# dtarb/TauDEM

Hardware: AMD Instinct MI355X
Metric: Mcells/s (PitRemove->D8FlowDir->AreaD8 pipeline) (higher is better)
Workload: dtype f32

## Files before the change

taudem_amd/csrc/aread8.hip:

```cpp
#include "context.hpp"
#include "device_common.hpp"
#include "d8_sweep.hpp"
#include "flats.hpp"
#include "strips.hpp"

#include <cstdlib>
#include <cstring>

namespace {
using namespace tdxk;

constexpr int32_t CNT_NOT_PART = 0x40000000;
constexpr int32_t CNT_SOURCE = -1;
constexpr int32_t CNT_DONE = -2;

constexpr int16_t P_OUTSIDE = 16, P_SINK = 32;

enum { D8X_SUM = 0, D8X_MAX = 1, D8X_MIN = 2 };
struct D8Expr { int mode; float out_nodata; };
__device__ __forceinline__ bool d8_participates(int16_t p, int16_t nodata) { return !is_nodata_s(p, nodata) && ((p >= 0 && p <= 8) || p == P_SINK); }

__device__ __forceinline__ int d8_indegree(const int16_t* __restrict__ P, int nx, int ny, int x, int y, int16_t nodata) {
    int cnt = 0;
#pragma unroll
// ... 175 lines not shown
                if (xn >= 0 && xn < nx && yn >= y_own0 && yn < y_own1) {
                    const size_t n = size_t(yn) * size_t(nx) + size_t(xn);
                    drain_stores();
                    const int32_t old = __hip_atomic_fetch_sub(&cnt[n], 1, __ATOMIC_ACQ_REL, __HIP_MEMORY_SCOPE_AGENT);
                    if (old == 1) ad8_walk_from(n, P, Wt, w_nodata, nx, ny, y_own0, y_own1, nodata, contcheck, cnt, A, ex);
                }
            }
        }
    }
    const unsigned long long m = __ballot(ch);
    if ((threadIdx.x & 63) == 0 && m) atomicAdd(nchanged, (unsigned long long)__popcll(m));
}


constexpr int TS = 64;
constexpr int TH = TS + 2;
static_assert(TS == 64, "S_TGT() shifts by 6");
constexpr uint32_t NODE_DEAD = 0xFFFFFFFEu;
constexpr uint32_t NEXT_NONE = 0xFFFFFFFFu;
constexpr uint32_t NEXT_REMOTE_UP = 0xFFFFFFFDu;
constexpr uint32_t NEXT_REMOTE_DOWN = 0xFFFFFFFCu;
constexpr unsigned long long BOX_VALID = 1ull << 63;
constexpr float BIG_MARK = -2.0f;

static __global__ __launch_bounds__(256) void ad8_init_kernel(unsigned long long* __restrict__ d_cnt, uint32_t* __restrict__ node_indeg, uint32_t* __restrict__ node_next, size_t nnodes,
                                                              unsigned long long* __restrict__ boxes, uint8_t* __restrict__ delivered, size_t nx) {
    const size_t i = size_t(blockIdx.x) * 256 + threadIdx.x;
    if (i < 8) d_cnt[i] = 0ull;
    if (i < nnodes) { node_indeg[i] = 0xFFFFFFFFu; node_next[i] = 0xFFFFFFFFu; }
    if (i < 4 * nx) boxes[i] = 0ull;
    if (i < 2 * nx) delivered[i] = 0;
}
struct Ad8Geom {
    int nx, ny_arr, y0, y1, tiles_x, tiles_y;
    uint32_t nnodes_local;
};
__device__ __forceinline__ int rows_valid(const Ad8Geom& g, int ty) { const int r = g.y1 - (g.y0 + ty * TS); return r < TS ? r : TS; }

__device__ __forceinline__ unsigned lw_pack(unsigned cnt, unsigned arr, unsigned con, unsigned poi, unsigned indeg) {
    return cnt | (arr << 13) | (con << 17) | (poi << 21) | (indeg << 25);
}
__device__ __forceinline__ unsigned lw_cnt(unsigned w) { return w & 0x1FFFu; }
__device__ __forceinline__ unsigned lw_arr(unsigned w) { return (w >> 13) & 15u; }
__device__ __forceinline__ unsigned lw_con(unsigned w) { return (w >> 17) & 15u; }
__device__ __forceinline__ unsigned lw_poi(unsigned w) { return (w >> 21) & 15u; }
__device__ __forceinline__ unsigned lw_indeg(unsigned w) { return (w >> 25) & 15u; }
__device__ __forceinline__ unsigned long long nw_pack(unsigned cnt, unsigned arr, unsigned con, unsigned poi) {
    return (unsigned long long)cnt | ((unsigned long long)arr << 32) | ((unsigned long long)con << 42) | ((unsigned long long)poi << 52);
}
__device__ __forceinline__ unsigned nw_arr(unsigned long long w) { return unsigned(w >> 32) & 1023u; }
__device__ __forceinline__ unsigned nw_con(unsigned long long w) { return unsigned(w >> 42) & 1023u; }
__device__ __forceinline__ unsigned nw_poi(unsigned long long w) { return unsigned(w >> 52) & 1023u; }
__device__ __forceinline__ uint32_t cw_pack(unsigned cnt, bool con, bool poi) { return cnt | (con ? 1u << 30 : 0u) | (poi ? 1u << 31 : 0u); }

__device__ __forceinline__ int perim_pos(int lx, int ly, int rv) {
    if (ly == 0) return lx;
    if (ly == rv - 1) return 64 + lx;
    if (lx == 0) return 128 + (ly - 1);
    return 190 + (ly - 1);
}
__device__ __forceinline__ uint32_t node_id(const Ad8Geom& g, int gx, int gy) {
    if (gy < g.y0) return g.nnodes_local + uint32_t(gx);
    if (gy >= g.y1) return g.nnodes_local + uint32_t(g.nx) + uint32_t(gx);
    const int ty = (gy - g.y0) / TS, ly = (gy - g.y0) % TS;
    return uint32_t(ty * g.tiles_x + gx / TS) * 256u + uint32_t(perim_pos(gx % TS, ly, rows_valid(g, ty)));
}


constexpr unsigned OH_NODATA = 0x8000u, OH_SINK = 0x4000u, OH_DIRS = 0x1FEu, OH_PART = 0x1FFu | OH_SINK;
__device__ __forceinline__ unsigned p_onehot(int v, int nodata) {
    const unsigned sel = v == nodata ? 15u : (v == int(P_SINK) ? 14u : (unsigned(v) <= 8u ? unsigned(v) : 31u));
    return (1u << sel) & (0x1FFu | OH_SINK | OH_NODATA);
}
__device__ __forceinline__ void stage_p_onehot(const int16_t* __restrict__ P, int nx, int ny_arr, int x0, int ya0, int16_t nodata, uint16_t* sO) {
    constexpr int NIT = (TH * TH + 255) / 256, HALF = (NIT + 1) / 2;
#pragma unroll
    for (int b = 0; b < 2; b++) {
        int16_t v[HALF];
        unsigned ok = 0;
#pragma unroll
        for (int i = 0; i < HALF; i++) {
            const int e = int(threadIdx.x) + (b * HALF + i) * 256, ec = e < TH * TH ? e : TH * TH - 1;
            const int ly = ec / TH, lx = ec - ly * TH;
            const int gx = x0 + lx - 1, gy = ya0 + ly - 1;
            const int gxc = gx < 0 ? 0 : (gx >= nx ? nx - 1 : gx), gyc = gy < 0 ? 0 : (gy >= ny_arr ? ny_arr - 1 : gy);
            v[i] = P[size_t(gyc) * size_t(nx) + size_t(gxc)];
            if (gx == gxc && gy == gyc) ok |= 1u << i;
        }
#pragma unroll
        for (int i = 0; i < HALF; i++) {
            const int e = int(threadIdx.x) + (b * HALF + i) * 256;
            if (b * HALF + i < NIT && e < TH * TH) sO[e] = uint16_t(((ok >> i) & 1u) ? p_onehot(int(v[i]), int(nodata)) : OH_NODATA);
        }
        __builtin_amdgcn_sched_barrier(0);
    }
}
__device__ __forceinline__ bool in_tile(int lx, int ly, int rv) { return lx >= 0 && lx < TS && ly >= 0 && ly < rv; }

__device__ __forceinline__ bool ring_cell(int j, int rv, int& hx, int& hy) {
    if (j < TH) { hx = j - 1; hy = -1; return true; }
    if (j < 2 * TH) { hx = j - TH - 1; hy = rv; return true; }
    j -= 2 * TH;
    if (j < rv) { hx = -1; hy = j; return true; }
    j -= rv;
    if (j < rv) { hx = TS; hy = j; return true; }
    return false;
// ... 117 lines not shown
    }
    __syncthreads();
    AD8_MARK(3);
    for (int j = tid; j < 4 * TH; j += 256) {
        int hx, hy;
        if (!ring_cell(j, rv, hx, hy)) continue;
        const unsigned dirs = sRing[j] & OH_DIRS;
        if (!dirs) continue;
        const int ph = __ffs(int(dirs)) - 1;
        const int vx = hx + d1(ph), vy = hy + d2(ph);
        if (!in_tile(vx, vy, rv)) continue;
        int cur = vy * TS + vx, hops = 0;
        if (lw_indeg(sAcc[cur]) == 15u) continue;
        while (S_TGT(cur) >= 0 && hops < TS * TS) { cur = S_TGT(cur); hops++; }
        uint32_t nxt = NEXT_NONE;
        if (S_TGT(cur) == -2) {
            const int pp = perim_pos(cur % TS, cur / TS, rv);
            atomicAdd(&sIn[pp], 1u);
            nxt = uint32_t(tile) * 256u + uint32_t(pp);
        }
        node_next[node_id(g, x0 + hx, ya0 + hy)] = nxt;
    }
    __syncthreads();
    AD8_MARK(4);
#pragma unroll
    for (int r = 0; r < 16; r++) {
        const int ly = ry0 + r, c = ly * TS + lx;
        const int gx = x0 + lx, gy = ya0 + ly;
        if (gx >= g.nx || ly >= rv) continue;
        const unsigned w = sAcc[c];
        const bool part = lw_indeg(w) != 15u;
        const bool complete = part && lw_arr(w) == lw_indeg(w);
        cellw[size_t(gy) * size_t(g.nx) + size_t(gx)] = part ? cw_pack(lw_cnt(w), lw_con(w) != 0u, lw_poi(w) != 0u || !complete) : 0u;
        if (part && tgt[r] == -2) {
            const int pp = perim_pos(lx, ly, rv);
            const uint32_t nid = uint32_t(tile) * 256u + uint32_t(pp);
            node_acc[nid] = nw_pack(lw_cnt(w), 0u, lw_con(w) ? 1u : 0u, lw_poi(w) ? 1u : 0u);
            node_indeg[nid] = complete ? sIn[pp] : NODE_DEAD;
            const int tgy = gy + (((exit_up >> r) & 1u) ? -1 : (((exit_down >> r) & 1u) ? 1 : 0));
            if (tgy < g.y0) node_next[nid] = NEXT_REMOTE_UP;
            else if (tgy >= g.y1) node_next[nid] = NEXT_REMOTE_DOWN;
        }
    }
#undef S_TGT
    if (DBG) {
        __syncthreads();
        AD8_MARK(5);
        if (tid == 0)
            for (int i = 0; i < 5; i++) atomicAdd(&g_ad8_dbg[i], tcs[i + 1] - tcs[i]);
    }
#undef AD8_MARK
}

__device__ __forceinline__ bool stage_p_raw(const int16_t* __restrict__ P, int nx, int ny_arr, int x0, int ya0, int16_t nodata, uint8_t* sC) {
    constexpr int NIT = (TH * TH + 255) / 256, HALF = (NIT + 1) / 2;
    bool bad = false;
#pragma unroll
    for (int b = 0; b < 2; b++) {
        int16_t v[HALF];
        unsigned ok = 0;
#pragma unroll
        for (int i = 0; i < HALF; i++) {
            const int e = int(threadIdx.x) + (b * HALF + i) * 256, ec = e < TH * TH ? e : TH * TH - 1;
            const int ly = ec / TH, lx = ec - ly * TH;
            const int gx = x0 + lx - 1, gy = ya0 + ly - 1;
            const int gxc = gx < 0 ? 0 : (gx >= nx ? nx - 1 : gx), gyc = gy < 0 ? 0 : (gy >= ny_arr ? ny_arr - 1 : gy);
            v[i] = P[size_t(gyc) * size_t(nx) + size_t(gxc)];
            if (gx == gxc && gy == gyc) ok |= 1u << i;
        }
#pragma unroll
        for (int i = 0; i < HALF; i++) {
            const int e = int(threadIdx.x) + (b * HALF + i) * 256;
            if (b * HALF + i < NIT && e < TH * TH) {
                const bool good = ((ok >> i) & 1u) && v[i] != nodata && unsigned(int(v[i]) - 1) < 8u;
                sC[e] = good ? uint8_t(v[i]) : uint8_t(0);
                bad |= !good;
            }
        }
        __builtin_amdgcn_sched_barrier(0);
    }
    return bad;
}

__device__ unsigned long long g_ad8_dbg_fast[8];
constexpr int AD8_MAX_ROUNDS = 12;
template <bool DBG>
__global__ __launch_bounds__(256, 6) void ad8_tile_fast_kernel(const int16_t* __restrict__ P, Ad8Geom g, int16_t nodata,
                                                            uint32_t* __restrict__ cellw, unsigned long long* __restrict__ node_acc,
                                                            uint32_t* __restrict__ node_indeg, uint32_t* __restrict__ node_next,
                                                            uint32_t* __restrict__ redo, unsigned long long* __restrict__ nredo) {
    unsigned long long tcs[6];
#define AD8_MARK(i) do { if (DBG) tcs[i] = clock64(); } while (0)
    AD8_MARK(0);
    __shared__ int16_t sT[TS * TS];
    __shared__ unsigned sAcc[TS * TS];
    __shared__ unsigned sIn[256];
    __shared__ unsigned sVote[3][4];
    static_assert(TH * TH <= int(sizeof(int16_t)) * TS * TS, "the staged codes fit the pointer table");
    uint8_t* const sC = reinterpret_cast<uint8_t*>(sT);
    const int tile = blockIdx.x;
    const int tx = tile % g.tiles_x, ty = tile / g.tiles_x;
    const int x0 = tx * TS, ya0 = g.y0 + ty * TS, rv = rows_valid(g, ty);
    const int tid = threadIdx.x, lx = tid & 63, ry0 = (tid >> 6) * 16, wave = tid >> 6;
    bool bad = rv != TS || x0 < 1 || x0 + TS >= g.nx || ya0 < 1 || ya0 + TS >= g.ny_arr;
    if (!bad) bad = stage_p_raw(P, g.nx, g.ny_arr, x0, ya0, nodata, sC);
    sIn[tid] = 0u;
    const bool wave_bad = __ballot(bad) != 0ull;
    if (lx == 0) sVote[0][wave] = wave_bad ? 1u : 0u;
    __syncthreads();
    if ((sVote[0][0] | sVote[0][1] | sVote[0][2] | sVote[0][3]) != 0u) {
        if (tid == 0) redo[atomicAdd(nredo, 1ull)] = uint32_t(tile);
        return;
    }
    AD8_MARK(1);
    unsigned exits = 0, exit_up = 0, exit_down = 0;
    int16_t ptr[16];
#pragma unroll
    for (int r = 0; r < 16; r++) {
        const int ly = ry0 + r;
        const int p = sC[(ly + 1) * TH + lx + 1];
        const int tlx = lx + d1(p), tly = ly + d2(p);
        const bool in = in_tile(tlx, tly, TS);
        ptr[r] = int16_t(in ? tly * TS + tlx : -2);
        if (!in) {
            exits |= 1u << r;
            if (d2(p) < 0) exit_up |= 1u << r;
            if (d2(p) > 0) exit_down |= 1u << r;
        }
    }
    int ent[2];
#pragma unroll
    for (int k = 0; k < 2; k++) {
        const int j = tid + 256 * k;
        int hx, hy;
        ent[k] = -1;
        if (j < 4 * TH && ring_cell(j, TS, hx, hy)) {
            const int ph = sC[(hy + 1) * TH + hx + 1];
            const int vx = hx + d1(ph), vy = hy + d2(ph);
            if (in_tile(vx, vy, TS)) ent[k] = vy * TS + vx;
        }
    }
    __syncthreads();
#pragma unroll
    for (int r = 0; r < 16; r++) {
        sT[(ry0 + r) * TS + lx] = ptr[r];
        sAcc[(ry0 + r) * TS + lx] = 1u;
    }
    __syncthreads();
    AD8_MARK(2);
    uint32_t ent_next[2];
#pragma unroll
    for (int k = 0; k < 2; k++) {
        ent_next[k] = NEXT_NONE;
        if (ent[k] < 0) continue;
        int cur = ent[k], hops = 0;
        while (sT[cur] >= 0 && hops < TS * TS) { cur = sT[cur]; hops++; }
        if (sT[cur] == -2) {
            const int pp = perim_pos(cur % TS, cur / TS, TS);
            atomicAdd(&sIn[pp], 1u);
            ent_next[k] = uint32_t(tile) * 256u + uint32_t(pp);
        }
    }
    __syncthreads();
    AD8_MARK(3);
    unsigned acc[16];
    unsigned live = ~exits & 0xFFFFu;
#pragma unroll
    for (int r = 0; r < 16; r++) acc[r] = 1u;
    int rounds = 0;
    for (;;) {
        int nn[16];
#pragma unroll
        for (int r = 0; r < 16; r++) nn[r] = sT[((live >> r) & 1u) ? int(ptr[r]) : (ry0 + r) * TS + lx];
#pragma unroll
        for (int r = 0; r < 16; r++)
            if ((live >> r) & 1u) (void)__hip_atomic_fetch_add(&sAcc[ptr[r]], acc[r], __ATOMIC_RELAXED, __HIP_MEMORY_SCOPE_WORKGROUP);
        __syncthreads();
#pragma unroll
        for (int r = 0; r < 16; r++)
            if ((live >> r) & 1u) {
                const int c = (ry0 + r) * TS + lx;
                ptr[r] = int16_t(nn[r]);
                sT[c] = int16_t(nn[r]);
                if (nn[r] < 0) live &= ~(1u << r);
                else acc[r] = sAcc[c];
            }
        rounds++;
        const bool wave_live = __ballot(live != 0u) != 0ull;
        if (lx == 0) sVote[1 + (rounds & 1)][wave] = wave_live ? 1u : 0u;
        __syncthreads();
        const unsigned* v = sVote[1 + (rounds & 1)];
        if ((v[0] | v[1] | v[2] | v[3]) == 0u) break;
        if (rounds == AD8_MAX_ROUNDS) {
            if (tid == 0) redo[atomicAdd(nredo, 1ull)] = uint32_t(tile);
            return;
        }
    }
    AD8_MARK(4);
#pragma unroll
    for (int k = 0; k < 2; k++) {
        const int j = tid + 256 * k;
        int hx, hy;
        if (ent[k] >= 0 && ring_cell(j, TS, hx, hy)) node_next[node_id(g, x0 + hx, ya0 + hy)] = ent_next[k];
    }
#pragma unroll
    for (int r = 0; r < 16; r++) {
        const int ly = ry0 + r, c = ly * TS + lx;
        const int gx = x0 + lx, gy = ya0 + ly;
        const unsigned cnt = sAcc[c];
        cellw[size_t(gy) * size_t(g.nx) + size_t(gx)] = cw_pack(cnt, false, false);
        if ((exits >> r) & 1u) {
            const int pp = perim_pos(lx, ly, TS);
            const uint32_t nid = uint32_t(tile) * 256u + uint32_t(pp);
            node_acc[nid] = nw_pack(cnt, 0u, 0u, 0u);
            node_indeg[nid] = sIn[pp];
            const int tgy = gy + (((exit_up >> r) & 1u) ? -1 : (((exit_down >> r) & 1u) ? 1 : 0));
            if (tgy < g.y0) node_next[nid] = NEXT_REMOTE_UP;
            else if (tgy >= g.y1) node_next[nid] = NEXT_REMOTE_DOWN;
        }
    }
    if (DBG) {
        __syncthreads();
        AD8_MARK(5);
        if (tid == 0) {
            for (int i = 0; i < 5; i++) atomicAdd(&g_ad8_dbg_fast[i], tcs[i + 1] - tcs[i]);
            atomicAdd(&g_ad8_dbg_fast[5], (unsigned long long)rounds);
            atomicAdd(&g_ad8_dbg_fast[6], 1ull);
        }
    }
#undef AD8_MARK
}

__device__ __forceinline__ void forest_walk_from(uint32_t u, unsigned long long w, const Ad8Geom& g, unsigned long long* __restrict__ node_acc,
                                                 const uint32_t* __restrict__ node_indeg, const uint32_t* __restrict__ node_next,
                                                 unsigned long long* __restrict__ outbox) {
    uint32_t n = node_next[u];
    for (;;) {
        if (n == NEXT_NONE) return;
        if (n == NEXT_REMOTE_UP || n == NEXT_REMOTE_DOWN) {
            const uint32_t tile = u >> 8, pos = u & 255u;
            const uint32_t gx = (tile % uint32_t(g.tiles_x)) * TS + (pos & 63u);
            outbox[(n == NEXT_REMOTE_UP ? 0u : uint32_t(g.nx)) + gx] = (w & ~BOX_VALID) | BOX_VALID;
            return;
        }
        const uint32_t nn = node_next[n], ind = node_indeg[n];
        const unsigned long long add = nw_pack(unsigned(w), 1u, nw_con(w) ? 1u : 0u, nw_poi(w) ? 1u : 0u);
        const unsigned long long nw = __hip_atomic_fetch_add(&node_acc[n], add, __ATOMIC_RELAXED, __HIP_MEMORY_SCOPE_AGENT) + add;
        if (nw_arr(nw) != ind) return;
        u = n; w = nw; n = nn;
    }
}

__global__ __launch_bounds__(256) void ad8_forest_walk_kernel(Ad8Geom g, unsigned long long* __restrict__ node_acc, const uint32_t* __restrict__ node_indeg,
                                                              const uint32_t* __restrict__ node_next, unsigned long long* __restrict__ outbox) {
    const size_t i = size_t(blockIdx.x) * 256 + threadIdx.x;
    if (i >= g.nnodes_local || node_indeg[i] != 0u) return;
    forest_walk_from(uint32_t(i), node_acc[i], g, node_acc, node_indeg, node_next, outbox);
}

__global__ __launch_bounds__(256) void ad8_forest_deliver_kernel(Ad8Geom g, const unsigned long long* __restrict__ inbox, uint8_t* __restrict__ delivered,
                                                                 unsigned long long* __restrict__ node_acc, uint32_t* __restrict__ node_indeg,
                                                                 const uint32_t* __restrict__ node_next, unsigned long long* __restrict__ outbox,
                                                                 unsigned long long* __restrict__ ndelivered) {
    const int i = blockIdx.x * 256 + threadIdx.x;
    bool did = false;
    if (i < 2 * g.nx) {
        const unsigned long long b = inbox[i];
        if ((b & BOX_VALID) && !delivered[i]) {
            delivered[i] = 1;
            did = true;
            const uint32_t hn = g.nnodes_local + uint32_t(i);
            const unsigned long long w = b & ~BOX_VALID;
            const unsigned long long hw = nw_pack(unsigned(w), 0u, nw_con(w) ? 1u : 0u, nw_poi(w) ? 1u : 0u);
            node_acc[hn] = hw;
            node_indeg[hn] = 0u;
            forest_walk_from(hn, hw, g, node_acc, node_indeg, node_next, outbox);
        }
    }
    const unsigned long long m = __ballot(did);
    if ((threadIdx.x & 63) == 0 && m) atomicAdd(ndelivered, (unsigned long long)__popcll(m));
}

__global__ __launch_bounds__(256) void ad8_tile_apply_kernel(const int16_t* __restrict__ P, Ad8Geom g, int16_t nodata,
                                                             uint32_t* __restrict__ cellw, const unsigned long long* __restrict__ node_acc,
                                                             const uint32_t* __restrict__ node_indeg, int contcheck, unsigned big_threshold,
                                                             float* __restrict__ A, uint32_t* __restrict__ biglist,
                                                             unsigned long long* __restrict__ nbig) {
    __shared__ uint16_t sO[TH * TH];
    __shared__ unsigned sCnt[TS * TS];
    __shared__ unsigned sFlag[TS * TS / 16];
    __shared__ uint16_t sRing[4 * TH];
    int16_t* const sT = reinterpret_cast<int16_t*>(sO);
    const int tile = blockIdx.x;
    const int tx = tile % g.tiles_x, ty = tile / g.tiles_x;
    const int x0 = tx * TS, ya0 = g.y0 + ty * TS, rv = rows_valid(g, ty);
    const int tid = threadIdx.x, lx = tid & 63, ry0 = (tid >> 6) * 16;
    stage_p_onehot(P, g.nx, g.ny_arr, x0, ya0, nodata, sO);
    sFlag[tid] = 0u;
    __syncthreads();
    for (int j = tid; j < 4 * TH; j += 256) {
        int hx, hy;
        sRing[j] = ring_cell(j, rv, hx, hy) ? sO[(hy + 1) * TH + hx + 1] : uint16_t(0);
    }
    int16_t tgt[16];
    unsigned partmask = 0;
    {
        uint32_t cw[16];
        unsigned oown[16], otgt[16];
        const int gx = x0 + lx, gxc = gx < g.nx ? gx : g.nx - 1;
#pragma unroll
        for (int r = 0; r < 16; r++) {
            const int ly = ry0 + r, lyc = ly < rv ? ly : rv - 1;
            cw[r] = cellw[size_t(ya0 + lyc) * size_t(g.nx) + size_t(gxc)];
        }
#pragma unroll
        for (int r = 0; r < 16; r++) oown[r] = sO[(ry0 + r + 1) * TH + lx + 1];
#pragma unroll
        for (int r = 0; r < 16; r++) {
            const unsigned dirs = oown[r] & OH_DIRS;
            const int pc = dirs ? __ffs(int(dirs)) - 1 : 1;
            otgt[r] = sO[(ry0 + r + d2(pc) + 1) * TH + lx + d1(pc) + 1];
        }
#pragma unroll
        for (int r = 0; r < 16; r++) {
            const int ly = ry0 + r;
            const unsigned dirs = oown[r] & OH_DIRS;
            const int p = dirs ? __ffs(int(dirs)) - 1 : 0;
            int t = -1;
            if (ly < rv && (oown[r] & OH_PART) != 0u) {
                partmask |= 1u << r;
                if (p >= 1) {
                    const int tlx = lx + d1(p), tly = ly + d2(p);
                    if (in_tile(tlx, tly, rv) && (otgt[r] & OH_PART) != 0u) t = tly * TS + tlx;
                }
            }
            tgt[r] = int16_t(t);
            const uint32_t w = (gx < g.nx && ly < rv) ? cw[r] : 0u;
            sCnt[ly * TS + lx] = w & 0x3FFFFFFFu;
            const unsigned fl = w >> 30;
            if (fl) atomicOr(&sFlag[(ly * TS + lx) >> 4], fl << (2 * ((ly * TS + lx) & 15)));
        }
    }
    __syncthreads();
#define S_TGT(c) sT[c]
#pragma unroll
    for (int r = 0; r < 16; r++) {
        if (ry0 + r < rv) sT[(ry0 + r) * TS + lx] = (tgt[r] >= 0) ? tgt[r] : (((partmask >> r) & 1u) ? int16_t(-3) : int16_t(-1));
    }
    __syncthreads();
    for (int j = tid; j < 4 * TH; j += 256) {
        int hx, hy;
        if (!ring_cell(j, rv, hx, hy)) continue;
        const unsigned dirs = sRing[j] & OH_DIRS;
        if (!dirs) continue;
        const int ph = __ffs(int(dirs)) - 1;
        const int vx = hx + d1(ph), vy = hy + d2(ph);
        if (!in_tile(vx, vy, rv)) continue;
        int cur = vy * TS + vx, hops = 0;
        if (S_TGT(cur) == -1) continue;
        const uint32_t nid = node_id(g, x0 + hx, ya0 + hy);
        const uint32_t ind = node_indeg[nid];
        const unsigned long long w = node_acc[nid];
        unsigned addc = 0, addf = 2u;
        if (ind < NODE_DEAD && nw_arr(w) == ind) { addc = unsigned(w); addf = (nw_con(w) ? 1u : 0u) | (nw_poi(w) ? 2u : 0u); }
        for (;;) {
            if (addc) __hip_atomic_fetch_add(&sCnt[cur], addc, __ATOMIC_RELAXED, __HIP_MEMORY_SCOPE_WORKGROUP);
            if (addf) atomicOr(&sFlag[cur >> 4], addf << (2 * (cur & 15)));
            const int t = S_TGT(cur);
            if (t < 0 || ++hops >= TS * TS) break;
            cur = t;
        }
    }
    __syncthreads();
    unsigned bigmask = 0;
#pragma unroll
    for (int r = 0; r < 16; r++) {
        const int ly = ry0 + r, c = ly * TS + lx;
        const int gx = x0 + lx, gy = ya0 + ly;
        if (gx >= g.nx || ly >= rv) continue;
        const unsigned cnt = sCnt[c];
        const unsigned fl = (sFlag[c >> 4] >> (2 * (c & 15))) & 3u;
        const bool part = (partmask >> r) & 1u;
        const bool con = (fl & 1u) != 0u, poi = (fl & 2u) != 0u;
        float a = TDX_AREA_NODATA;
        if (part && !poi && !(con && contcheck == 1)) {
            if (cnt > big_threshold) { a = BIG_MARK; bigmask |= 1u << r; cellw[size_t(gy) * size_t(g.nx) + size_t(gx)] = cnt; }
            else a = (float)cnt;
        }
        A[size_t(gy) * size_t(g.nx) + size_t(gx)] = a;
    }
#undef S_TGT
    const unsigned long long pos0 = block_reserve(unsigned(__popc(bigmask)), nbig);
    unsigned long long pos = pos0;
#pragma unroll
    for (int r = 0; r < 16; r++)
        if (bigmask & (1u << r)) biglist[pos++] = uint32_t(size_t(ya0 + ry0 + r) * size_t(g.nx) + size_t(x0 + lx));
}

__global__ __launch_bounds__(256) void ad8_big_keys_kernel(const uint32_t* __restrict__ biglist, unsigned long long nbig, const uint32_t* __restrict__ cellw,
                                                           uint32_t* __restrict__ keys) {
    const unsigned long long q = (unsigned long long)blockIdx.x * 256 + threadIdx.x;
    if (q < nbig) keys[q] = cellw[biglist[q]];
}
__global__ __launch_bounds__(256) void ad8_big_pos_kernel(const uint32_t* __restrict__ sorted, const unsigned long long* __restrict__ nbig_dev, uint32_t* __restrict__ pos) {
    const unsigned long long q = (unsigned long long)blockIdx.x * 256 + threadIdx.x;
    if (q < *nbig_dev) pos[sorted[q]] = uint32_t(q);
}
__global__ __launch_bounds__(1024) void ad8_big_compact_kernel(const uint32_t* __restrict__ in, const uint32_t* __restrict__ root_in, const unsigned long long* __restrict__ nin_dev,
                                                               const float* __restrict__ A, uint32_t* __restrict__ out, uint32_t* __restrict__ root_out,
                                                               unsigned long long* __restrict__ nout) {
    __shared__ unsigned wsum[16];
    const unsigned long long n = *nin_dev;
    const int lane = threadIdx.x & 63, w = threadIdx.x >> 6;
    unsigned long long base = 0;
    for (unsigned long long q0 = 0; q0 < n; q0 += 1024) {
        const unsigned long long q = q0 + threadIdx.x;
        const uint32_t cell = q < n ? in[q] : 0u;
        const bool keep = q < n && A[cell] == BIG_MARK;
        const unsigned long long m = __ballot(keep);
        if (lane == 0) wsum[w] = unsigned(__popcll(m));
        __syncthreads();
        unsigned before = 0, total = 0;
#pragma unroll
        for (int i = 0; i < 16; i++) { const unsigned v = wsum[i]; before += i < w ? v : 0u; total += v; }
        if (keep) {
            const unsigned long long o = base + before + unsigned(__popcll(m & ((1ull << lane) - 1ull)));
            out[o] = cell;
            root_out[o] = root_in[q];
        }
        base += total;
        __syncthreads();
    }
    if (threadIdx.x == 0) *nout = base;
}

__global__ __launch_bounds__(256) void ad8_big_next_kernel(const int16_t* __restrict__ P, int nx, int y_own0, int y_own1, const uint32_t* __restrict__ sorted,
                                                           unsigned long long nbig, const uint32_t* __restrict__ pos, const float* __restrict__ A,
                                                           uint32_t* __restrict__ nxt) {
    const unsigned long long q = (unsigned long long)blockIdx.x * 256 + threadIdx.x;
    if (q >= nbig) return;
    const size_t c = size_t(sorted[q]);
    const int x = int(c % size_t(nx)), y = int(c / size_t(nx));
    const int p = P[c];
    uint32_t r = uint32_t(q);
    if (p >= 1 && p <= 8) {
        const int xn = x + d1(p), yn = y + d2(p);
        if (xn >= 0 && xn < nx && yn >= y_own0 && yn < y_own1) {
            const size_t n = size_t(yn) * size_t(nx) + size_t(xn);
            if (A[n] == BIG_MARK) r = pos[n];
// ... 221 lines not shown
                const float v = __builtin_bit_cast(float, __builtin_amdgcn_readlane(__builtin_bit_cast(int, result), j));
                if (lane == i) a8[k] = v;
            }
            if (lane == i) result = fold();
        }
        if (q < nbig) s_big[base + unsigned(lane)] = pending ? result : own;
        base = base + 64u >= ring ? 0u : base + 64u;
        if (pending && result != BIG_MARK) {
            if (spill) st_agent(&bigval[q], result);
            A[cell] = result;
            done++;
        }
        if (spill && (((chunk0 - b0) >> 6) & 63ull) == 63ull) drain_stores();
        else if (spill && ring < 64u * 130u) drain_stores();
        {
            const float last = __builtin_bit_cast(float, __builtin_amdgcn_readlane(__builtin_bit_cast(int, result), 63));
            if (last >= 1.0f) hint = last;
        }
    }
    }
    if (done) atomicAdd(nfinal, done);
}


}


int tdx_sort_pairs_u32(tdx_context* ctx, int scratch_slot, const uint32_t* keys_in, uint32_t* keys_out, const uint32_t* vals_in, uint32_t* vals_out,
                       size_t n);

static int aread8_tiled(tdx_context* ctx, const Strip& st, int16_t* d_p, int16_t p_nodata, int contcheck, float* d_ad8, tdx_stats* stats) {
    hipStream_t s = ctx->stream;
    const int inx = st.nx;
    const size_t n = size_t(st.nx) * size_t(st.ny_arr);
    Ad8Geom g;
    g.nx = st.nx; g.ny_arr = st.ny_arr; g.y0 = st.y0; g.y1 = st.y1;
    g.tiles_x = (st.nx + TS - 1) / TS; g.tiles_y = (st.y1 - st.y0 + TS - 1) / TS;
    const size_t ntiles = size_t(g.tiles_x) * size_t(g.tiles_y);
    g.nnodes_local = uint32_t(ntiles * 256);
    const size_t nnodes = size_t(g.nnodes_local) + 2 * size_t(st.nx);
    uint32_t* cellw = static_cast<uint32_t*>(ctx->scratch(TDX_S_A, n * 4));
    unsigned long long* node_acc = static_cast<unsigned long long*>(ctx->scratch(TDX_S_B, nnodes * 8));
    uint32_t* node_indeg = static_cast<uint32_t*>(ctx->scratch(TDX_S_C, nnodes * 4));
    uint32_t* node_next = static_cast<uint32_t*>(ctx->scratch(TDX_S_D, nnodes * 4));
    const unsigned big_threshold = getenv("TDX_AD8_BIG_THRESHOLD") ? unsigned(atol(getenv("TDX_AD8_BIG_THRESHOLD"))) : (1u << 24);
    const size_t bigcap = big_threshold < (1u << 24) ? n : n / 8 + 4096;
    uint32_t* biglist = static_cast<uint32_t*>(ctx->scratch(TDX_S_E, bigcap * 4));
    unsigned long long* boxes = static_cast<unsigned long long*>(ctx->scratch(TDX_S_F, size_t(st.nx) * 4 * 8));
    uint8_t* delivered = static_cast<uint8_t*>(ctx->scratch(TDX_S_G, size_t(st.nx) * 2));
    uint32_t* redo = static_cast<uint32_t*>(ctx->scratch(TDX_S_K, ntiles * 4));
    if (!cellw || !node_acc || !node_indeg || !node_next || !biglist || !boxes || !delivered || !redo) return TDX_ERR_NOMEM;
    const char* const ad8_local = getenv("TDX_AD8_LOCAL");
    const bool kahn_only = ad8_local && strcmp(ad8_local, "kahn") == 0;
    unsigned long long *outbox = boxes, *inbox = boxes + 2 * size_t(st.nx);
    unsigned long long* d_cnt = reinterpret_cast<unsigned long long*>(ctx->d_mail);
    unsigned long long* nredo = d_cnt + 7;
    ctx->begin_call(stats);
    strip_mark(ctx, st, "aread8");
    int rc = strip_exchange<int16_t>(ctx, st, d_p, p_nodata);
    if (rc != TDX_OK) return rc;
    hipLaunchKernelGGL(ad8_init_kernel, dim3(tdx_blocks_for(std::max(nnodes, size_t(st.nx) * 4), 256)), dim3(256), 0, s, d_cnt, node_indeg, node_next, nnodes, boxes,
                       delivered, size_t(st.nx));
    {
        TdxSpan sp(ctx, TDX_K_STENCIL);
        static const bool ad8_debug = getenv("TDX_AD8_DEBUG") != nullptr;
        const unsigned nt = unsigned(ntiles);
        const uint32_t* list = kahn_only ? nullptr : redo;
        if (ad8_debug) {
            unsigned long long z[8] = {}, zf[8] = {};
            TDX_HIP_CHECK(ctx, hipMemcpyToSymbol(HIP_SYMBOL(g_ad8_dbg), z, sizeof(z)));
            TDX_HIP_CHECK(ctx, hipMemcpyToSymbol(HIP_SYMBOL(g_ad8_dbg_fast), zf, sizeof(zf)));
            if (!kahn_only)
                hipLaunchKernelGGL((ad8_tile_fast_kernel<true>), dim3(nt), dim3(256), 0, s, d_p, g, p_nodata, cellw, node_acc, node_indeg, node_next, redo, nredo);
            hipLaunchKernelGGL((ad8_tile_local_kernel<true, true>), dim3(nt), dim3(256), 0, s, d_p, g, p_nodata, cellw, node_acc, node_indeg, node_next, list, nredo);
            TDX_HIP_CHECK(ctx, hipStreamSynchronize(s));
            TDX_HIP_CHECK(ctx, hipMemcpyFromSymbol(z, HIP_SYMBOL(g_ad8_dbg), sizeof(z)));
            TDX_HIP_CHECK(ctx, hipMemcpyFromSymbol(zf, HIP_SYMBOL(g_ad8_dbg_fast), sizeof(zf)));
            unsigned long long nr = ntiles;
            if (!kahn_only) TDX_HIP_CHECK(ctx, hipMemcpy(&nr, nredo, sizeof(nr), hipMemcpyDeviceToHost));
            const double nk = double(nr ? nr : 1), nf = double(zf[6] ? zf[6] : 1);
            fprintf(stderr, "ad8_tile_local: %llu tiles, cycles per tile: stage %.0f, topology %.0f, targets %.0f, Kahn walks %.0f, entry walks %.0f, write-back %.0f\n", nr,
                    double(z[0]) / nk, double(z[1]) / nk, 0.0, double(z[2]) / nk, double(z[3]) / nk, double(z[4]) / nk);
            if (!kahn_only)
                fprintf(stderr, "ad8_tile_fast: %llu tiles, cycles per tile: stage %.0f, targets %.0f, entry walks %.0f, doubling %.0f, write-back %.0f; %.2f rounds per tile\n", zf[6],
                        double(zf[0]) / nf, double(zf[1]) / nf, double(zf[2]) / nf, double(zf[3]) / nf, double(zf[4]) / nf, double(zf[5]) / nf);
        } else {
            if (!kahn_only)
                hipLaunchKernelGGL((ad8_tile_fast_kernel<false>), dim3(nt), dim3(256), 0, s, d_p, g, p_nodata, cellw, node_acc, node_indeg, node_next, redo, nredo);
            if (getenv("TDX_AD8_KAHN_NESTED"))
                hipLaunchKernelGGL((ad8_tile_local_kernel<false, false>), dim3(nt), dim3(256), 0, s, d_p, g, p_nodata, cellw, node_acc, node_indeg, node_next, list, nredo);
            else
                hipLaunchKernelGGL((ad8_tile_local_kernel<false, true>), dim3(nt), dim3(256), 0, s, d_p, g, p_nodata, cellw, node_acc, node_indeg, node_next, list, nredo);
        }
        if (stats) stats->launches[TDX_K_STENCIL] += kahn_only ? 1 : 2;
    }
    int64_t outer = 1;
    ctx->phase = "forest";
    {
        TdxSpan sp(ctx, TDX_K_ACCUM);
        hipLaunchKernelGGL(ad8_forest_walk_kernel, dim3(tdx_blocks_for(size_t(g.nnodes_local), 256)), dim3(256), 0, s, g, node_acc, node_indeg, node_next,
                           outbox);
        if (stats) stats->launches[TDX_K_ACCUM]++;
        while (st.multi()) {
            const size_t rowb = size_t(st.nx) * 8;
            rc = strip_exchange_buffers(ctx, st, outbox, outbox + st.nx, inbox, inbox + st.nx, rowb);
            if (rc != TDX_OK) return rc;
            TDX_HIP_CHECK(ctx, hipMemsetAsync(d_cnt + 1, 0, sizeof(unsigned long long), s));
            hipLaunchKernelGGL(ad8_forest_deliver_kernel, dim3(tdx_blocks_for(size_t(2 * st.nx), 256)), dim3(256), 0, s, g, inbox, delivered, node_acc,
                               node_indeg, node_next, outbox, d_cnt + 1);
            int64_t got = 0;
            rc = strip_allreduce_device(ctx, st, d_cnt + 1, 1, TDX_OP_SUM, &got);
            if (rc != TDX_OK) return rc;
            if (stats) stats->launches[TDX_K_ACCUM]++;
            if (got == 0) break;
            outer++;
        }
    }
    const int64_t outer_forest = outer;
    ctx->phase = "apply";
    {
        TdxSpan sp(ctx, TDX_K_STENCIL);
        hipLaunchKernelGGL(ad8_tile_apply_kernel, dim3(unsigned(ntiles)), dim3(256), 0, s, d_p, g, p_nodata, cellw, node_acc, node_indeg, contcheck,
                           big_threshold, d_ad8, biglist, d_cnt);
        if (stats) stats->launches[TDX_K_STENCIL]++;
    }
    TDX_HIP_CHECK(ctx, hipMemcpyAsync(ctx->h_mail, d_cnt, 8 * sizeof(unsigned long long), hipMemcpyDeviceToHost, s));
    TDX_HIP_CHECK(ctx, hipStreamSynchronize(s));
    const unsigned long long nbig = ctx->h_mail[0];
    ctx->ad8_redo_tiles = kahn_only ? int64_t(ntiles) : int64_t(ctx->h_mail[7]);
    ctx->ad8_fast_tiles = int64_t(ntiles) - ctx->ad8_redo_tiles;
    if (nbig > bigcap) return tdx_fail(ctx, TDX_ERR_NOMEM, "AreaD8: big-cell list exhausted");
    int64_t nbig_all = int64_t(nbig);
    rc = strip_allreduce(ctx, st, &nbig_all, 1, TDX_OP_SUM);
    if (rc != TDX_OK) return rc;
    ctx->phase = "big cells";
    if (nbig_all > 0) {
        TdxSpan sp(ctx, TDX_K_MISC);
        const size_t nb1 = size_t(nbig ? nbig : 1);
        uint32_t* keys = static_cast<uint32_t*>(ctx->scratch(TDX_S_H, (nb1 * 8 + 4) * 4));
        if (!keys) return TDX_ERR_NOMEM;
        uint32_t *keys_sorted = keys + nb1, *sorted = keys_sorted + nb1, *rootA = sorted + nb1, *rootB = rootA + nb1, *grouped = rootB + nb1, *listB = grouped + nb1,
                 *segbeg = listB + nb1;
        uint32_t* pos = cellw;
        const bool no_trees = getenv("TDX_AD8_BIG_ONE_WAVE") != nullptr;
        static const bool no_incremental = getenv("TDX_AD8_BIG_FULL_ROUNDS") != nullptr;
        const int big_scan = getenv("TDX_AD8_BIG_SCAN") ? std::max(0, atoi(getenv("TDX_AD8_BIG_SCAN"))) : 4;
        const unsigned big_ring = getenv("TDX_AD8_BIG_RING") ? std::min(BIG_LDS, std::max(64u, unsigned(atoi(getenv("TDX_AD8_BIG_RING"))) / 64u * 64u)) : BIG_LDS;
        uint32_t *cur = sorted, *cur_root = rootA, *other = listB, *other_root = rootB;
        unsigned long long* n_cur = d_cnt;
        const unsigned gb = tdx_blocks_for(nb1, 256);
        if (nbig) {
            hipLaunchKernelGGL(ad8_big_keys_kernel, dim3(gb), dim3(256), 0, s, biglist, nbig, cellw, keys);
            rc = tdx_sort_pairs_u32(ctx, TDX_S_I, keys, keys_sorted, biglist, sorted, size_t(nbig));
            if (rc != TDX_OK) return rc;
            if (!no_trees) {
                hipLaunchKernelGGL(ad8_big_pos_kernel, dim3(gb), dim3(256), 0, s, sorted, n_cur, pos);
                hipLaunchKernelGGL(ad8_big_next_kernel, dim3(gb), dim3(256), 0, s, d_p, inx, st.y0, st.y1, sorted, nbig, pos, d_ad8, rootA);
                uint32_t *ra = rootA, *rb = rootB;
                for (unsigned long long reach = 1; reach < nbig; reach *= 2) {
                    hipLaunchKernelGGL(ad8_big_jump_kernel, dim3(gb), dim3(256), 0, s, ra, rb, nbig);
                    std::swap(ra, rb);
                }
                rc = tdx_sort_pairs_u32(ctx, TDX_S_I, ra, keys, sorted, grouped, size_t(nbig));
                if (rc != TDX_OK) return rc;
                cur = grouped; cur_root = keys; other = listB; other_root = keys_sorted;
            }
        }
        float* big_vals = static_cast<float*>(ctx->scratch(TDX_S_J, nb1 * 4 * 18));
        if (!big_vals) return TDX_ERR_NOMEM;
        uint32_t* big_deps = reinterpret_cast<uint32_t*>(big_vals) + nb1 * 8;
        uint32_t* big_flags = big_deps + nb1 * 8;
        float* big_val = reinterpret_cast<float*>(big_flags + nb1);
        rc = strip_exchange<float>(ctx, st, d_ad8, TDX_AREA_NODATA);
        if (rc != TDX_OK) return rc;
        int flip = 0;
        for (;;) {
            if (nbig) {
// ... 264 lines not shown
```

Baseline: 12990.

## Add fast apply path for clean AreaD8 tiles using codes packed into cell words

The fast tile kernel now loads pointer codes straight into registers instead of staging a haloed tile in shared memory. It defers root finding to after pointer doubling, using complemented self-indices as root markers. It stores each cell's direction code next to its count in the cell word, so a new apply kernel can finish clean tiles from those words and the ring codes alone, while the full apply kernel runs only over the redo tile list. This skips re-staging and rebuilding topology for most tiles, at the cost of an extra launch, more code paths, and a device-side read of the redo count in every full-apply block.

```diff
diff --git a/taudem_amd/csrc/aread8.hip b/taudem_amd/csrc/aread8.hip
--- a/taudem_amd/csrc/aread8.hip
+++ b/taudem_amd/csrc/aread8.hip
@@ -251,6 +251,10 @@
 __device__ __forceinline__ unsigned nw_con(unsigned long long w) { return unsigned(w >> 42) & 1023u; }
 __device__ __forceinline__ unsigned nw_poi(unsigned long long w) { return unsigned(w >> 52) & 1023u; }
 __device__ __forceinline__ uint32_t cw_pack(unsigned cnt, bool con, bool poi) { return cnt | (con ? 1u << 30 : 0u) | (poi ? 1u << 31 : 0u); }
+constexpr int CW_CODE_SHIFT = 13;
+constexpr uint32_t CW_CODE_MASK = 15u << CW_CODE_SHIFT, CW_FAST_CNT_MASK = (1u << CW_CODE_SHIFT) - 1u;
+static_assert((CW_CODE_MASK & (CW_FAST_CNT_MASK | (1u << 30) | (1u << 31))) == 0u && CW_FAST_CNT_MASK >= 4096u, "the code field touches neither a clean tile's count nor the flags");
+__device__ __forceinline__ unsigned cw_code(uint32_t w) { return (w & CW_CODE_MASK) >> CW_CODE_SHIFT; }
 
 __device__ __forceinline__ int perim_pos(int lx, int ly, int rv) {
     if (ly == 0) return lx;
@@ -474,34 +478,12 @@
 #undef AD8_MARK
 }
 
-__device__ __forceinline__ bool stage_p_raw(const int16_t* __restrict__ P, int nx, int ny_arr, int x0, int ya0, int16_t nodata, uint8_t* sC) {
-    constexpr int NIT = (TH * TH + 255) / 256, HALF = (NIT + 1) / 2;
-    bool bad = false;
-#pragma unroll
-    for (int b = 0; b < 2; b++) {
-        int16_t v[HALF];
-        unsigned ok = 0;
-#pragma unroll
-        for (int i = 0; i < HALF; i++) {
-            const int e = int(threadIdx.x) + (b * HALF + i) * 256, ec = e < TH * TH ? e : TH * TH - 1;
-            const int ly = ec / TH, lx = ec - ly * TH;
-            const int gx = x0 + lx - 1, gy = ya0 + ly - 1;
-            const int gxc = gx < 0 ? 0 : (gx >= nx ? nx - 1 : gx), gyc = gy < 0 ? 0 : (gy >= ny_arr ? ny_arr - 1 : gy);
-            v[i] = P[size_t(gyc) * size_t(nx) + size_t(gxc)];
-            if (gx == gxc && gy == gyc) ok |= 1u << i;
-        }
-#pragma unroll
-        for (int i = 0; i < HALF; i++) {
-            const int e = int(threadIdx.x) + (b * HALF + i) * 256;
-            if (b * HALF + i < NIT && e < TH * TH) {
-                const bool good = ((ok >> i) & 1u) && v[i] != nodata && unsigned(int(v[i]) - 1) < 8u;
-                sC[e] = good ? uint8_t(v[i]) : uint8_t(0);
-                bad |= !good;
-            }
-        }
-        __builtin_amdgcn_sched_barrier(0);
-    }
-    return bad;
+__device__ __forceinline__ bool ad8_code_good(int16_t v, int16_t nodata) { return v != nodata && unsigned(int(v) - 1) < 8u; }
+__device__ __forceinline__ bool ring_slot(int tid, int k, int& hx, int& hy) {
+    const int j = tid + 256 * k;
+    const bool has = j < 2 * TH + 2 * TS;
+    (void)ring_cell(has ? j : 2 * TH + 2 * TS - 1, TS, hx, hy);
+    return has;
 }
 
 __device__ unsigned long long g_ad8_dbg_fast[8];
@@ -510,7 +492,7 @@
 __global__ __launch_bounds__(256, 6) void ad8_tile_fast_kernel(const int16_t* __restrict__ P, Ad8Geom g, int16_t nodata,
                                                             uint32_t* __restrict__ cellw, unsigned long long* __restrict__ node_acc,
                                                             uint32_t* __restrict__ node_indeg, uint32_t* __restrict__ node_next,
-                                                            uint32_t* __restrict__ redo, unsigned long long* __restrict__ nredo) {
+                                                            uint32_t* __restrict__ redo, unsigned long long* __restrict__ nredo, unsigned mark) {
     unsigned long long tcs[6];
 #define AD8_MARK(i) do { if (DBG) tcs[i] = clock64(); } while (0)
     AD8_MARK(0);
@@ -518,15 +500,28 @@
     __shared__ unsigned sAcc[TS * TS];
     __shared__ unsigned sIn[256];
     __shared__ unsigned sVote[3][4];
-    static_assert(TH * TH <= int(sizeof(int16_t)) * TS * TS, "the staged codes fit the pointer table");
-    uint8_t* const sC = reinterpret_cast<uint8_t*>(sT);
+    __shared__ uint8_t sRc[256];
     const int tile = blockIdx.x;
     const int tx = tile % g.tiles_x, ty = tile / g.tiles_x;
     const int x0 = tx * TS, ya0 = g.y0 + ty * TS, rv = rows_valid(g, ty);
-    const int tid = threadIdx.x, lx = tid & 63, ry0 = (tid >> 6) * 16, wave = tid >> 6;
-    bool bad = rv != TS || x0 < 1 || x0 + TS >= g.nx || ya0 < 1 || ya0 + TS >= g.ny_arr;
-    if (!bad) bad = stage_p_raw(P, g.nx, g.ny_arr, x0, ya0, nodata, sC);
+    const int tid = threadIdx.x, lx = tid & 63, wave = __builtin_amdgcn_readfirstlane(tid >> 6), ry0 = wave * 16;
+    if (rv != TS || x0 < 1 || x0 + TS >= g.nx || ya0 < 1 || ya0 + TS >= g.ny_arr) {
+        if (tid == 0) redo[atomicAdd(nredo, 1ull)] = uint32_t(tile);
+        return;
+    }
+    int16_t pc[16], pr[2];
+#pragma unroll
+    for (int r = 0; r < 16; r++) pc[r] = (P + (size_t(ya0 + ry0 + r) * size_t(g.nx) + size_t(x0)))[unsigned(lx)];
+#pragma unroll
+    for (int k = 0; k < 2; k++) {
+        int hx, hy;
+        (void)ring_slot(tid, k, hx, hy);
+        pr[k] = P[size_t(ya0 + hy) * size_t(g.nx) + size_t(x0 + hx)];
+    }
     sIn[tid] = 0u;
+    bool bad = !ad8_code_good(pr[0], nodata) || !ad8_code_good(pr[1], nodata);
+#pragma unroll
+    for (int r = 0; r < 16; r++) bad |= !ad8_code_good(pc[r], nodata);
     const bool wave_bad = __ballot(bad) != 0ull;
     if (lx == 0) sVote[0][wave] = wave_bad ? 1u : 0u;
     __syncthreads();
@@ -535,55 +530,22 @@
         return;
     }
     AD8_MARK(1);
-    unsigned exits = 0, exit_up = 0, exit_down = 0;
+    unsigned exits = 0;
     int16_t ptr[16];
 #pragma unroll
     for (int r = 0; r < 16; r++) {
         const int ly = ry0 + r;
-        const int p = sC[(ly + 1) * TH + lx + 1];
+        const int p = pc[r];
         const int tlx = lx + d1(p), tly = ly + d2(p);
         const bool in = in_tile(tlx, tly, TS);
-        ptr[r] = int16_t(in ? tly * TS + tlx : -2);
-        if (!in) {
-            exits |= 1u << r;
-            if (d2(p) < 0) exit_up |= 1u << r;
-            if (d2(p) > 0) exit_down |= 1u << r;
-        }
-    }
-    int ent[2];
-#pragma unroll
-    for (int k = 0; k < 2; k++) {
-        const int j = tid + 256 * k;
-        int hx, hy;
-        ent[k] = -1;
-        if (j < 4 * TH && ring_cell(j, TS, hx, hy)) {
-            const int ph = sC[(hy + 1) * TH + hx + 1];
-            const int vx = hx + d1(ph), vy = hy + d2(ph);
-            if (in_tile(vx, vy, TS)) ent[k] = vy * TS + vx;
-        }
-    }
-    __syncthreads();
-#pragma unroll
-    for (int r = 0; r < 16; r++) {
-        sT[(ry0 + r) * TS + lx] = ptr[r];
-        sAcc[(ry0 + r) * TS + lx] = 1u;
-    }
+        ptr[r] = int16_t(in ? tly * TS + tlx : ~(ly * TS + lx));
+        if (!in) exits |= 1u << r;
+        sT[ly * TS + lx] = ptr[r];
+        sAcc[ly * TS + lx] = 1u | (unsigned(p) << CW_CODE_SHIFT);
+    }
+    sRc[tid] = uint8_t(unsigned(pr[0]) | (unsigned(pr[1]) << 4));
     __syncthreads();
     AD8_MARK(2);
-    uint32_t ent_next[2];
-#pragma unroll
-    for (int k = 0; k < 2; k++) {
-        ent_next[k] = NEXT_NONE;
-        if (ent[k] < 0) continue;
-        int cur = ent[k], hops = 0;
-        while (sT[cur] >= 0 && hops < TS * TS) { cur = sT[cur]; hops++; }
-        if (sT[cur] == -2) {
-            const int pp = perim_pos(cur % TS, cur / TS, TS);
-            atomicAdd(&sIn[pp], 1u);
-            ent_next[k] = uint32_t(tile) * 256u + uint32_t(pp);
-        }
-    }
-    __syncthreads();
     AD8_MARK(3);
     unsigned acc[16];
     unsigned live = ~exits & 0xFFFFu;
@@ -605,7 +567,7 @@
                 ptr[r] = int16_t(nn[r]);
                 sT[c] = int16_t(nn[r]);
                 if (nn[r] < 0) live &= ~(1u << r);
-                else acc[r] = sAcc[c];
+                else acc[r] = sAcc[c] & CW_FAST_CNT_MASK;
             }
         rounds++;
         const bool wave_live = __ballot(live != 0u) != 0ull;
@@ -619,24 +581,36 @@
         }
     }
     AD8_MARK(4);
+    int tid_again = tid;
+    asm volatile("" : "+v"(tid_again));
+    const int lxw = tid_again & 63;
+    const unsigned rcodes = sRc[tid_again];
 #pragma unroll
     for (int k = 0; k < 2; k++) {
-        const int j = tid + 256 * k;
         int hx, hy;
-        if (ent[k] >= 0 && ring_cell(j, TS, hx, hy)) node_next[node_id(g, x0 + hx, ya0 + hy)] = ent_next[k];
-    }
+        const bool has = ring_slot(tid_again, k, hx, hy);
+        const int ph = int((rcodes >> (4 * k)) & 15u);
+        const int vx = hx + d1(ph), vy = hy + d2(ph);
+        if (!has || !in_tile(vx, vy, TS)) continue;
+        const int root = ~int(sT[vy * TS + vx]);
+        const int pp = perim_pos(root % TS, root / TS, TS);
+        atomicAdd(&sIn[pp], 1u);
+        node_next[node_id(g, x0 + hx, ya0 + hy)] = uint32_t(tile) * 256u + uint32_t(pp);
+    }
+    __syncthreads();
 #pragma unroll
     for (int r = 0; r < 16; r++) {
-        const int ly = ry0 + r, c = ly * TS + lx;
+        const int lx = lxw, ly = ry0 + r, c = ly * TS + lx;
         const int gx = x0 + lx, gy = ya0 + ly;
-        const unsigned cnt = sAcc[c];
-        cellw[size_t(gy) * size_t(g.nx) + size_t(gx)] = cw_pack(cnt, false, false);
-        if ((exits >> r) & 1u) {
+        const unsigned w = sAcc[c], cnt = w & CW_FAST_CNT_MASK;
+        const int p = int(cw_code(w));
+        cellw[size_t(gy) * size_t(g.nx) + size_t(gx)] = mark ? w : cw_pack(cnt, false, false);
+        if (!in_tile(lx + d1(p), ly + d2(p), TS)) {
             const int pp = perim_pos(lx, ly, TS);
             const uint32_t nid = uint32_t(tile) * 256u + uint32_t(pp);
             node_acc[nid] = nw_pack(cnt, 0u, 0u, 0u);
             node_indeg[nid] = sIn[pp];
-            const int tgy = gy + (((exit_up >> r) & 1u) ? -1 : (((exit_down >> r) & 1u) ? 1 : 0));
+            const int tgy = gy + d2(p);
             if (tgy < g.y0) node_next[nid] = NEXT_REMOTE_UP;
             else if (tgy >= g.y1) node_next[nid] = NEXT_REMOTE_DOWN;
         }
@@ -703,23 +677,31 @@
     if ((threadIdx.x & 63) == 0 && m) atomicAdd(ndelivered, (unsigned long long)__popcll(m));
 }
 
+__device__ unsigned long long g_ad8_dbg_apply[16];
+template <bool DBG>
 __global__ __launch_bounds__(256) void ad8_tile_apply_kernel(const int16_t* __restrict__ P, Ad8Geom g, int16_t nodata,
                                                              uint32_t* __restrict__ cellw, const unsigned long long* __restrict__ node_acc,
                                                              const uint32_t* __restrict__ node_indeg, int contcheck, unsigned big_threshold,
                                                              float* __restrict__ A, uint32_t* __restrict__ biglist,
-                                                             unsigned long long* __restrict__ nbig) {
+                                                             unsigned long long* __restrict__ nbig,
+                                                             const uint32_t* __restrict__ list, const unsigned long long* __restrict__ nlist) {
+    if (list && blockIdx.x >= *nlist) return;
+    unsigned long long tcs[5];
+#define AD8_MARK(i) do { if (DBG) tcs[i] = clock64(); } while (0)
+    AD8_MARK(0);
     __shared__ uint16_t sO[TH * TH];
     __shared__ unsigned sCnt[TS * TS];
     __shared__ unsigned sFlag[TS * TS / 16];
     __shared__ uint16_t sRing[4 * TH];
     int16_t* const sT = reinterpret_cast<int16_t*>(sO);
-    const int tile = blockIdx.x;
+    const int tile = list ? int(list[blockIdx.x]) : int(blockIdx.x);
     const int tx = tile % g.tiles_x, ty = tile / g.tiles_x;
     const int x0 = tx * TS, ya0 = g.y0 + ty * TS, rv = rows_valid(g, ty);
     const int tid = threadIdx.x, lx = tid & 63, ry0 = (tid >> 6) * 16;
     stage_p_onehot(P, g.nx, g.ny_arr, x0, ya0, nodata, sO);
     sFlag[tid] = 0u;
     __syncthreads();
+    AD8_MARK(1);
     for (int j = tid; j < 4 * TH; j += 256) {
         int hx, hy;
         sRing[j] = ring_cell(j, rv, hx, hy) ? sO[(hy + 1) * TH + hx + 1] : uint16_t(0);
@@ -770,6 +752,7 @@
         if (ry0 + r < rv) sT[(ry0 + r) * TS + lx] = (tgt[r] >= 0) ? tgt[r] : (((partmask >> r) & 1u) ? int16_t(-3) : int16_t(-1));
     }
     __syncthreads();
+    AD8_MARK(2);
     for (int j = tid; j < 4 * TH; j += 256) {
         int hx, hy;
         if (!ring_cell(j, rv, hx, hy)) continue;
@@ -794,6 +777,7 @@
         }
     }
     __syncthreads();
+    AD8_MARK(3);
     unsigned bigmask = 0;
 #pragma unroll
     for (int r = 0; r < 16; r++) {
@@ -817,6 +801,107 @@
 #pragma unroll
     for (int r = 0; r < 16; r++)
         if (bigmask & (1u << r)) biglist[pos++] = uint32_t(size_t(ya0 + ry0 + r) * size_t(g.nx) + size_t(x0 + lx));
+    if (DBG) {
+        __syncthreads();
+        AD8_MARK(4);
+        if (tid == 0) {
+            for (int i = 0; i < 4; i++) atomicAdd(&g_ad8_dbg_apply[i], tcs[i + 1] - tcs[i]);
+            atomicAdd(&g_ad8_dbg_apply[4], 1ull);
+        }
+    }
+#undef AD8_MARK
+}
+
+template <bool DBG>
+__global__ __launch_bounds__(256, 6) void ad8_tile_apply_fast_kernel(const int16_t* __restrict__ P, Ad8Geom g, uint32_t* __restrict__ cellw,
+                                                                  const unsigned long long* __restrict__ node_acc, const uint32_t* __restrict__ node_indeg,
+                                                                  int contcheck, unsigned big_threshold, float* __restrict__ A, uint32_t* __restrict__ biglist,
+                                                                  unsigned long long* __restrict__ nbig) {
+    unsigned long long tcs[5];
+#define AD8_MARK(i) do { if (DBG) tcs[i] = clock64(); } while (0)
+    AD8_MARK(0);
+    __shared__ int16_t sT[TS * TS];
+    __shared__ unsigned sCnt[TS * TS];
+    __shared__ unsigned sFlag[TS * TS / 16];
+    const int tile = blockIdx.x;
+    const int tx = tile % g.tiles_x, ty = tile / g.tiles_x;
+    const int x0 = tx * TS, ya0 = g.y0 + ty * TS;
+    const int tid = threadIdx.x, lx = tid & 63, ry0 = __builtin_amdgcn_readfirstlane(tid >> 6) * 16;
+    if (rows_valid(g, ty) != TS || x0 < 1 || x0 + TS >= g.nx || ya0 < 1 || ya0 + TS >= g.ny_arr) return;
+    uint32_t cw[16];
+    int16_t pr[2];
+    int rhx[2], rhy[2];
+    bool rhas[2];
+#pragma unroll
+    for (int r = 0; r < 16; r++) cw[r] = (cellw + (size_t(ya0 + ry0 + r) * size_t(g.nx) + size_t(x0)))[unsigned(lx)];
+#pragma unroll
+    for (int k = 0; k < 2; k++) {
+        rhas[k] = ring_slot(tid, k, rhx[k], rhy[k]);
+        pr[k] = P[size_t(ya0 + rhy[k]) * size_t(g.nx) + size_t(x0 + rhx[k])];
+    }
+    if (cw_code(cw[0]) == 0u) return;
+    AD8_MARK(1);
+    sFlag[tid] = 0u;
+#pragma unroll
+    for (int r = 0; r < 16; r++) {
+        const int ly = ry0 + r;
+        const int p = int(cw_code(cw[r]));
+        const int tlx = lx + d1(p), tly = ly + d2(p);
+        sT[ly * TS + lx] = int16_t(in_tile(tlx, tly, TS) ? tly * TS + tlx : -1);
+        sCnt[ly * TS + lx] = cw[r] & CW_FAST_CNT_MASK;
+    }
+    __syncthreads();
+    AD8_MARK(2);
+#pragma unroll
+    for (int k = 0; k < 2; k++) {
+        const int ph = pr[k];
+        const int vx = rhx[k] + d1(ph), vy = rhy[k] + d2(ph);
+        if (!rhas[k] || !in_tile(vx, vy, TS)) continue;
+        int cur = vy * TS + vx, hops = 0;
+        const uint32_t nid = node_id(g, x0 + rhx[k], ya0 + rhy[k]);
+        const uint32_t ind = node_indeg[nid];
+        const unsigned long long w = node_acc[nid];
+        unsigned addc = 0, addf = 2u;
+        if (ind < NODE_DEAD && nw_arr(w) == ind) { addc = unsigned(w); addf = (nw_con(w) ? 1u : 0u) | (nw_poi(w) ? 2u : 0u); }
+        for (;;) {
+            if (addc) __hip_atomic_fetch_add(&sCnt[cur], addc, __ATOMIC_RELAXED, __HIP_MEMORY_SCOPE_WORKGROUP);
+            if (addf) atomicOr(&sFlag[cur >> 4], addf << (2 * (cur & 15)));
+            const int t = sT[cur];
+            if (t < 0 || ++hops >= TS * TS) break;
+            cur = t;
+        }
+    }
+    __syncthreads();
+    AD8_MARK(3);
+    unsigned bigmask = 0;
+#pragma unroll
+    for (int r = 0; r < 16; r++) {
+        const int ly = ry0 + r, c = ly * TS + lx;
+        const size_t idx = size_t(ya0 + ly) * size_t(g.nx) + size_t(x0 + lx);
+        const unsigned cnt = sCnt[c];
+        const unsigned fl = (sFlag[c >> 4] >> (2 * (c & 15))) & 3u;
+        const bool con = (fl & 1u) != 0u, poi = (fl & 2u) != 0u;
+        float a = TDX_AREA_NODATA;
+        if (!poi && !(con && contcheck == 1)) {
+            if (cnt > big_threshold) { a = BIG_MARK; bigmask |= 1u << r; cellw[idx] = cnt; }
+            else a = (float)cnt;
+        }
+        A[idx] = a;
+    }
+    const unsigned long long pos0 = block_reserve(unsigned(__popc(bigmask)), nbig);
+    unsigned long long pos = pos0;
+#pragma unroll
+    for (int r = 0; r < 16; r++)
+        if (bigmask & (1u << r)) biglist[pos++] = uint32_t(size_t(ya0 + ry0 + r) * size_t(g.nx) + size_t(x0 + lx));
+    if (DBG) {
+        __syncthreads();
+        AD8_MARK(4);
+        if (tid == 0) {
+            for (int i = 0; i < 4; i++) atomicAdd(&g_ad8_dbg_apply[8 + i], tcs[i + 1] - tcs[i]);
+            atomicAdd(&g_ad8_dbg_apply[12], 1ull);
+        }
+    }
+#undef AD8_MARK
 }
 
 __global__ __launch_bounds__(256) void ad8_big_keys_kernel(const uint32_t* __restrict__ biglist, unsigned long long nbig, const uint32_t* __restrict__ cellw,
@@ -1144,6 +1229,9 @@
     if (!cellw || !node_acc || !node_indeg || !node_next || !biglist || !boxes || !delivered || !redo) return TDX_ERR_NOMEM;
     const char* const ad8_local = getenv("TDX_AD8_LOCAL");
     const bool kahn_only = ad8_local && strcmp(ad8_local, "kahn") == 0;
+    const char* const ad8_apply = getenv("TDX_AD8_APPLY");
+    const bool apply_fast = !kahn_only && !(ad8_apply && strcmp(ad8_apply, "full") == 0);
+    const unsigned mark = apply_fast ? 1u : 0u;
     unsigned long long *outbox = boxes, *inbox = boxes + 2 * size_t(st.nx);
     unsigned long long* d_cnt = reinterpret_cast<unsigned long long*>(ctx->d_mail);
     unsigned long long* nredo = d_cnt + 7;
@@ -1163,7 +1251,7 @@
             TDX_HIP_CHECK(ctx, hipMemcpyToSymbol(HIP_SYMBOL(g_ad8_dbg), z, sizeof(z)));
             TDX_HIP_CHECK(ctx, hipMemcpyToSymbol(HIP_SYMBOL(g_ad8_dbg_fast), zf, sizeof(zf)));
             if (!kahn_only)
-                hipLaunchKernelGGL((ad8_tile_fast_kernel<true>), dim3(nt), dim3(256), 0, s, d_p, g, p_nodata, cellw, node_acc, node_indeg, node_next, redo, nredo);
+                hipLaunchKernelGGL((ad8_tile_fast_kernel<true>), dim3(nt), dim3(256), 0, s, d_p, g, p_nodata, cellw, node_acc, node_indeg, node_next, redo, nredo, mark);
             hipLaunchKernelGGL((ad8_tile_local_kernel<true, true>), dim3(nt), dim3(256), 0, s, d_p, g, p_nodata, cellw, node_acc, node_indeg, node_next, list, nredo);
             TDX_HIP_CHECK(ctx, hipStreamSynchronize(s));
             TDX_HIP_CHECK(ctx, hipMemcpyFromSymbol(z, HIP_SYMBOL(g_ad8_dbg), sizeof(z)));
@@ -1174,11 +1262,11 @@
             fprintf(stderr, "ad8_tile_local: %llu tiles, cycles per tile: stage %.0f, topology %.0f, targets %.0f, Kahn walks %.0f, entry walks %.0f, write-back %.0f\n", nr,
                     double(z[0]) / nk, double(z[1]) / nk, 0.0, double(z[2]) / nk, double(z[3]) / nk, double(z[4]) / nk);
             if (!kahn_only)
-                fprintf(stderr, "ad8_tile_fast: %llu tiles, cycles per tile: stage %.0f, targets %.0f, entry walks %.0f, doubling %.0f, write-back %.0f; %.2f rounds per tile\n", zf[6],
+                fprintf(stderr, "ad8_tile_fast: %llu tiles, cycles per tile: load and vote %.0f, targets %.0f, entry walks %.0f, doubling %.0f, roots and write-back %.0f; %.2f rounds per tile\n", zf[6],
                         double(zf[0]) / nf, double(zf[1]) / nf, double(zf[2]) / nf, double(zf[3]) / nf, double(zf[4]) / nf, double(zf[5]) / nf);
         } else {
             if (!kahn_only)
-                hipLaunchKernelGGL((ad8_tile_fast_kernel<false>), dim3(nt), dim3(256), 0, s, d_p, g, p_nodata, cellw, node_acc, node_indeg, node_next, redo, nredo);
+                hipLaunchKernelGGL((ad8_tile_fast_kernel<false>), dim3(nt), dim3(256), 0, s, d_p, g, p_nodata, cellw, node_acc, node_indeg, node_next, redo, nredo, mark);
             if (getenv("TDX_AD8_KAHN_NESTED"))
                 hipLaunchKernelGGL((ad8_tile_local_kernel<false, false>), dim3(nt), dim3(256), 0, s, d_p, g, p_nodata, cellw, node_acc, node_indeg, node_next, list, nredo);
             else
@@ -1212,9 +1300,31 @@
     ctx->phase = "apply";
     {
         TdxSpan sp(ctx, TDX_K_STENCIL);
-        hipLaunchKernelGGL(ad8_tile_apply_kernel, dim3(unsigned(ntiles)), dim3(256), 0, s, d_p, g, p_nodata, cellw, node_acc, node_indeg, contcheck,
-                           big_threshold, d_ad8, biglist, d_cnt);
-        if (stats) stats->launches[TDX_K_STENCIL]++;
+        static const bool ad8_debug = getenv("TDX_AD8_DEBUG") != nullptr;
+        const unsigned nt = unsigned(ntiles);
+        const uint32_t* list = apply_fast ? redo : nullptr;
+        if (ad8_debug) {
+            unsigned long long z[16] = {};
+            TDX_HIP_CHECK(ctx, hipMemcpyToSymbol(HIP_SYMBOL(g_ad8_dbg_apply), z, sizeof(z)));
+            if (apply_fast)
+                hipLaunchKernelGGL((ad8_tile_apply_fast_kernel<true>), dim3(nt), dim3(256), 0, s, d_p, g, cellw, node_acc, node_indeg, contcheck, big_threshold, d_ad8, biglist, d_cnt);
+            hipLaunchKernelGGL((ad8_tile_apply_kernel<true>), dim3(nt), dim3(256), 0, s, d_p, g, p_nodata, cellw, node_acc, node_indeg, contcheck, big_threshold, d_ad8, biglist,
+                               d_cnt, list, nredo);
+            TDX_HIP_CHECK(ctx, hipStreamSynchronize(s));
+            TDX_HIP_CHECK(ctx, hipMemcpyFromSymbol(z, HIP_SYMBOL(g_ad8_dbg_apply), sizeof(z)));
+            const double na = double(z[4] ? z[4] : 1), nf = double(z[12] ? z[12] : 1);
+            fprintf(stderr, "ad8_tile_apply: %llu tiles, cycles per tile: stage %.0f, topology %.0f, entry walks %.0f, write-back %.0f\n", z[4], double(z[0]) / na, double(z[1]) / na,
+                    double(z[2]) / na, double(z[3]) / na);
+            if (apply_fast)
+                fprintf(stderr, "ad8_tile_apply_fast: %llu tiles, cycles per tile: load %.0f, targets %.0f, entry walks %.0f, write-back %.0f\n", z[12], double(z[8]) / nf,
+                        double(z[9]) / nf, double(z[10]) / nf, double(z[11]) / nf);
+        } else {
+            if (apply_fast)
+                hipLaunchKernelGGL((ad8_tile_apply_fast_kernel<false>), dim3(nt), dim3(256), 0, s, d_p, g, cellw, node_acc, node_indeg, contcheck, big_threshold, d_ad8, biglist, d_cnt);
+            hipLaunchKernelGGL((ad8_tile_apply_kernel<false>), dim3(nt), dim3(256), 0, s, d_p, g, p_nodata, cellw, node_acc, node_indeg, contcheck, big_threshold, d_ad8, biglist,
+                               d_cnt, list, nredo);
+        }
+        if (stats) stats->launches[TDX_K_STENCIL] += apply_fast ? 2 : 1;
     }
     TDX_HIP_CHECK(ctx, hipMemcpyAsync(ctx->h_mail, d_cnt, 8 * sizeof(unsigned long long), hipMemcpyDeviceToHost, s));
     TDX_HIP_CHECK(ctx, hipStreamSynchronize(s));
```

Result: faster. 13400 (median of 6 runs) (+3.1%).
